# ignaschuemer7/soft-actor-critic

Hardware: NVIDIA B200
Metric: SAC updates/s (higher is better)
Workload: dtype f32

## Files before the change

### soft-actor-critic_b200/csrc/sacx.cu

```cuda
#include "../../include/sacx.h"

#include <cuda_runtime.h>

#include <cmath>
#include <cstdlib>
#include <cstring>
#include <string>
#include <vector>

#include "sacx_engine.cuh"
#include "sacx_per.cuh"

namespace sacx {

thread_local std::string g_err;
int fail(int code, const std::string& msg) {
  g_err = msg;
  return code;
}

constexpr int STAGE_ROWS = 4096;

struct Ring {
  int O, A, n_agents, W;
// ... 435 lines not shown
              if (pass == 1)
                ok = ok && tc_encode(enc, &g.maps.c[j], e->d_tc_scratch + r.part, n_ld, (uint64_t)t.splits * m_pad, n_ld, 32, TC_BM, 0, NA, sstride);
            }
            t.idesc = (1u << 4) | (2u << 7) | (2u << 10) | ((uint32_t)t.a_mn << 15) | ((uint32_t)t.b_mn << 16) |
                      ((uint32_t)(t.n_mma >> 3) << 17) | ((uint32_t)(TC_BM >> 4) << 24);
            t.tile0 = tiles; t.ntiles = t.m_tiles * t.splits;
            tiles += t.ntiles;
          }
          g.p.tiles_per_agent = tiles;
          g.p.total_tiles = tiles * (int)NA;
          g.grid = std::max(1, std::min(g.p.total_tiles, e->n_sms));
        }
        need = std::max(need, so);
      }
    }
    if (!ok) return off("cuTensorMapEncodeTiled rejected an operand layout");
    if (pass == 0) {
      sstride = (uint64_t)((need + 63) / 64 * 64 + 64);
      e->tc_scratch_floats = (size_t)sstride * NA;
      SACX_CUDA(cudaMalloc((void**)&e->d_tc_scratch, e->tc_scratch_floats * sizeof(float)));
      SACX_CUDA(cudaMemset(e->d_tc_scratch, 0, e->tc_scratch_floats * sizeof(float)));
    }
  }
  return SACX_OK;
}

static int engine_setup_rp_tma(Engine* e) {
  if (!e->rp) return SACX_OK;
  RpProgram& P = e->h_prog;
  Plan& plan = e->h_plans[PLAN_RP];
  void* fn = nullptr;
  cudaDriverEntryPointQueryResult qres;
  const bool have = cudaGetDriverEntryPoint("cuTensorMapEncodeTiled", &fn, cudaEnableDefault, &qres) == cudaSuccess && fn;
  std::vector<CUtensorMap> maps(P.n_jobs + 2 * plan.n_ops);
  memset(maps.data(), 0, sizeof(CUtensorMap) * maps.size());
  bool ok = have;
  for (int j = 0; ok && j < P.n_jobs; ++j) {
    const RpJob& jb = P.jobs[j];
    if (!jb.tma) continue;
    cuuint64_t dims[2], strides[1] = {(cuuint64_t)jb.w_ld * 4};
    cuuint32_t box[2], estr[2] = {1, 1};
    box[0] = 32; box[1] = 32;
    if (!jb.bkm) { dims[0] = jb.K; dims[1] = jb.N; }
    else { dims[0] = jb.N; dims[1] = jb.K; }
    ok = ((TcEncodeFn)fn)(&maps[j], CU_TENSOR_MAP_DATA_TYPE_FLOAT32, 2, e->arena + jb.w, dims, strides, box, estr, CU_TENSOR_MAP_INTERLEAVE_NONE,
                          CU_TENSOR_MAP_SWIZZLE_128B, CU_TENSOR_MAP_L2_PROMOTION_L2_128B, CU_TENSOR_MAP_FLOAT_OOB_FILL_NONE) == CUDA_SUCCESS;
  }
  if (!ok) { for (int j = 0; j < P.n_jobs; ++j) P.jobs[j].tma = 0; cudaGetLastError(); }
  const char* dw_env = getenv("SACX_RP_DW_TMA");
  bool ok_dw = have && !(dw_env && atoi(dw_env) == 0);
  for (int k = 0; k < plan.n_ops; ++k) { plan.ops[k].i[2] = 0; plan.ops[k].i[3] = 0; }
  for (int k = 0; ok_dw && k < plan.n_ops; ++k) {
    Op& o = plan.ops[k];
    if (o.type != OP_GEMM || o.epi != EPI_DW || o.a_sm != 1 || o.b_sn != 1 || (o.a & 3) || (o.b & 3) || (o.a_sk & 3) || (o.b_sk & 3)) continue;
    if (o.K > RP_DW_MAXK || o.cfg != 0) continue;
    for (int w = 0; ok_dw && w < 2; ++w) {
      cuuint64_t dims[2] = {(cuuint64_t)(w ? o.N : o.M), (cuuint64_t)o.K}, strides[1] = {(cuuint64_t)(w ? o.b_sk : o.a_sk) * 4};
      cuuint32_t box[2] = {32, (cuuint32_t)RP_DW_CHUNK}, estr[2] = {1, 1};
      ok_dw = ((TcEncodeFn)fn)(&maps[P.n_jobs + 2 * k + w], CU_TENSOR_MAP_DATA_TYPE_FLOAT32, 2, e->arena + (w ? o.b : o.a), dims, strides, box, estr,
                               CU_TENSOR_MAP_INTERLEAVE_NONE, CU_TENSOR_MAP_SWIZZLE_128B, CU_TENSOR_MAP_L2_PROMOTION_L2_128B,
                               CU_TENSOR_MAP_FLOAT_OOB_FILL_NONE) == CUDA_SUCCESS;
    }
    if (ok_dw) { o.i[2] = P.n_jobs + 2 * k + 1; o.i[3] = P.n_jobs + 2 * k + 2; }
  }
  if (!ok_dw) { for (int k = 0; k < plan.n_ops; ++k) { plan.ops[k].i[2] = 0; plan.ops[k].i[3] = 0; } cudaGetLastError(); }
  const char* vec_env = getenv("SACX_RP_DW_VEC");
  if (ok_dw && !(vec_env && atoi(vec_env) == 0)) {
    for (int k = 0; k < plan.n_ops; ++k) {
      Op& o = plan.ops[k];
      o.i[5] = 0;
      if (o.type == OP_GEMM && o.epi == EPI_DW && o.i[3] > 0 && o.M == 1 && o.K <= RP_DWV_MAXK && o.N >= 64 && !(o.flags & DW_ATOMIC) && o.i[0] <= 1) {
        o.i[5] = 1; o.tiles_n = (o.N + RP_DWV_COLS - 1) / RP_DWV_COLS; o.ntiles = o.tiles_n;
      }
    }
    int widest = 0;
    for (int ph = 0; ph < plan.n_phases; ++ph) {
      Phase& p = plan.phases[ph];
      p.ntiles = 0;
      for (int k = p.op0; k < p.op0 + p.nops; ++k) { plan.ops[k].tile0 = p.ntiles; p.ntiles += plan.ops[k].ntiles; }
      widest = std::max(widest, p.ntiles);
    }
    e->rp_grid = std::min(e->n_sms, std::max(e->rp_grid, widest));
  }
  if (e->d_rp_maps) { cudaFree(e->d_rp_maps); e->d_rp_maps = nullptr; }
  bool up = cudaMalloc(&e->d_rp_maps, sizeof(CUtensorMap) * maps.size()) == cudaSuccess;
  up = up && cudaMemcpy(e->d_rp_maps, maps.data(), sizeof(CUtensorMap) * maps.size(), cudaMemcpyHostToDevice) == cudaSuccess;
  if (!up) {
    for (int j = 0; j < P.n_jobs; ++j) P.jobs[j].tma = 0;
    for (int k = 0; k < plan.n_ops; ++k) { plan.ops[k].i[2] = 0; plan.ops[k].i[3] = 0; }
    if (e->d_rp_maps) { cudaFree(e->d_rp_maps); e->d_rp_maps = nullptr; }
    cudaGetLastError();
  }
  SACX_CUDA(cudaMemcpy(e->d_prog, &e->h_prog, sizeof(RpProgram), cudaMemcpyHostToDevice));
  return SACX_OK;
}

// ... 1126 lines not shown
```

### soft-actor-critic_b200/csrc/sacx_engine.cuh

```cuda
#pragma once
#include <cuda_runtime.h>

#include <algorithm>
#include <cstddef>
#include <cstdio>
#include <cstring>
#include <string>
#include <vector>

#include "sacx_kernels.cuh"
#include "sacx_rowpar.cuh"
#include "sacx_tc.cuh"

namespace sacx {

extern thread_local std::string g_err;
int fail(int code, const std::string& msg);
#define SACX_CUDA(call)                                                                        \
  do {                                                                                         \
    cudaError_t e__ = (call);                                                                  \
    if (e__ != cudaSuccess)                                                                    \
      return fail(SACX_ERR_CUDA, std::string(#call) + ": " + cudaGetErrorString(e__));         \
  } while (0)

// ... 749 lines not shown
    if (L - 2 - k >= 0) {
      const int l = L - 1 - k;
      pb.add(gemm_da(n, l, delta[l], ldd(l), delta[l - 1], ldd(l - 1), as.aux(l - 1), as.ld[l - 1]));
    }
    const int lw = L - k;
    if (lw >= 1 && !(skip_head_dw && lw == L))
      pb.add(gemm_dw(n, lw, opt, flags, delta[lw], ldd(lw), as.h[lw - 1], as.ld[lw - 1], is_critic));
    if (k == bwd_stages(n) - 1) pb.add(gemm_dw(n, 0, opt, flags, delta[0], ldd(0), x, ld_x, is_critic));
  }

  bool rowpar_eligible(std::string& why) const {
    const char* env = getenv("SACX_ROWPAR");
    if (env && atoi(env) == 0) { why = "disabled by SACX_ROWPAR=0"; return false; }
    if (cfg.n_agents != 1) { why = "population mode"; return false; }
    if (cfg.dp_world > 1) { why = "data-parallel mode"; return false; }
    { std::string w; if (tc_wanted(w)) { why = "large batch runs the tensor-core path"; return false; } }
    if (cfg.batch_size > 512 && !(env && atoi(env) == 1)) { why = "batch above 512: the tile-parallel kernel is faster"; return false; }
    if (pi.L() < 2 || q1.L() < 2) { why = "fewer than two hidden layers"; return false; }
    if (act_needs_z(pi.act_h) || act_needs_z(q1.act_h)) { why = "hidden activation needs saved pre-activations"; return false; }
    if (cfg.act_dim > RP_MAXA) { why = "action dimension above 8"; return false; }
    if (2 * cfg.obs_dim + cfg.act_dim + 2 > 256) { why = "observation wider than 123"; return false; }
    for (const NetLayout* n : {&pi, &q1})
      for (int l = 1; l <= n->L(); ++l)
        if (n->dims[l] != 64 && n->dims[l] != 128 && n->dims[l] != 256) { why = "hidden width not 64/128/256"; return false; }
    if (2 * (q1.L() + 1) + (pi.L() + 1) + 1 > RP_MAX_DW_OPS) { why = "network too deep"; return false; }
    return true;
  }

  bool build_rowpar(PB& pb) {
    RpProgram& P = h_prog;
    memset(&P, 0, sizeof P);
    const int O = cfg.obs_dim, A = cfg.act_dim, Lq = q1.L(), Lp = pi.L();
    bool overflow = false;
    int wmax = 0;
    auto step = [&](int row_op) {
      if (P.n_steps_a + P.n_steps_c >= RP_MAX_STEPS) { overflow = true; return; }
      RpStep& st = P.steps[P.n_steps_a + P.n_steps_c];
      st.row_op = row_op; st.job0 = P.n_jobs; st.njobs = 0; st.load0 = P.n_loads; st.nloads = 0;
    };
    auto cur = [&]() -> RpStep& { return P.steps[P.n_steps_a + P.n_steps_c]; };
    auto add_job = [&](const RpJob& j) {
      if (P.n_jobs >= RP_MAX_JOBS) { overflow = true; return; }
      const int NS = j.N / RP_CS;
      RpJob jj = j;
      jj.tma = (rp_tma && NS == 32 && (j.w_ld % 4) == 0 && (j.w % 4) == 0 && j.K <= 256) ? 1 : 0;
      jj.map = P.n_jobs;
      P.jobs[P.n_jobs++] = jj; cur().njobs++;
      const int cp_floats = j.bkm ? j.K * NS : NS * (j.Kp + 4);
      const int tma_floats = j.bkm ? j.K * 32 : ((j.K + 31) / 32) * 1024;
      wmax = std::max(wmax, jj.tma ? tma_floats : cp_floats);
    };
    auto add_load = [&](i64 off, int ld, int K, int abuf) {
      if (P.n_loads >= RP_MAX_LOADS) { overflow = true; return; }
      P.loads[P.n_loads++] = RpLoad{off, ld, K, abuf, 0}; cur().nloads++;
    };
    auto fwd = [&](const NetLayout& n, int l, i64 wshift, int a_src, const ActSet& as, int slot) {
      RpJob j; memset(&j, 0, sizeof j);
      j.bkm = 0; j.a_src = a_src; j.K = n.dims[l]; j.Kp = (j.K + 7) & ~7; j.N = n.dims[l + 1]; j.act = n.act_h;
      j.ns_log2 = j.N == 256 ? 5 : (j.N == 128 ? 4 : 3);
      j.w = n.W[l] + wshift; j.w_ld = j.K; j.bias = n.b[l] + wshift; j.out = as.h[l]; j.out_ld = as.ld[l]; j.aux = -1; j.proj_w = -1;
      if (l == n.L() - 1) {
        j.proj_J = n.dims[n.L() + 1]; j.proj_slot = slot; j.proj_w = n.W[n.L()] + wshift; j.proj_sj = n.dims[n.L()]; j.proj_sn = 1;
      }
      return j;
    };
    auto bwd = [&](const NetLayout& n, int l, int a_src, const ActSet& as, const i64* delta, int da_slot) {
      RpJob j; memset(&j, 0, sizeof j);
      j.bkm = 1; j.a_src = a_src; j.K = n.dims[l + 1]; j.Kp = j.K; j.N = n.dims[l]; j.act = n.act_h;
      j.ns_log2 = j.N == 256 ? 5 : (j.N == 128 ? 4 : 3);
      j.w = n.W[l]; j.w_ld = n.dims[l]; j.bias = -1; j.aux = as.h[l - 1]; j.aux_ld = as.ld[l - 1];
      j.out = delta[l - 1]; j.out_ld = rup4(n.dims[l]); j.proj_w = -1;
      if (da_slot >= 0) { j.proj_J = A; j.proj_slot = da_slot; j.proj_w = n.W[0] + O; j.proj_sj = 1; j.proj_sn = n.dims[0]; }
      return j;
    };
    const i64 tsh = T0 - q1.begin;
    step(RPR_GATHER);
    add_job(fwd(pi, 0, 0, RPS_XS2, a_pit, RPP_PI_T));
    add_job(fwd(pi, 0, 0, RPS_XSA, a_pia, RPP_PI_A));
    for (int c = 0; c < 2; ++c) add_job(fwd(c ? q2 : q1, 0, 0, RPS_XSA, a_q[c], RPP_Q1 + c));
    P.n_steps_a++;
    for (int l = 1; l < std::max(Lp, Lq); ++l) {
      step(RPR_NONE);
      if (l < Lp) {
        add_load(a_pit.h[l - 1], a_pit.ld[l - 1], pi.dims[l], 0); add_job(fwd(pi, l, 0, 0, a_pit, RPP_PI_T));
        add_load(a_pia.h[l - 1], a_pia.ld[l - 1], pi.dims[l], 1); add_job(fwd(pi, l, 0, 1, a_pia, RPP_PI_A));
      }
      if (l < Lq)
        for (int c = 0; c < 2; ++c) {
          add_load(a_q[c].h[l - 1], a_q[c].ld[l - 1], q1.dims[l], 2 + c);
          add_job(fwd(c ? q2 : q1, l, 0, 2 + c, a_q[c], RPP_Q1 + c));
        }
      P.n_steps_a++;
    }
    step(RPR_PI_HEADS);
    for (int c = 0; c < 2; ++c) add_job(fwd(c ? q2 : q1, 0, tsh, RPS_XS2, a_qt[c], RPP_QT1 + c));
    P.n_steps_a++;
    for (int l = 1; l < Lq; ++l) {
      step(RPR_NONE);
      for (int c = 0; c < 2; ++c) {
        add_load(a_qt[c].h[l - 1], a_qt[c].ld[l - 1], q1.dims[l], c);
        add_job(fwd(c ? q2 : q1, l, tsh, c, a_qt[c], RPP_QT1 + c));
      }
      P.n_steps_a++;
    }
    step(RPR_TARGET_CRITIC);
    for (int c = 0; c < 2; ++c) {
      add_load(a_q[c].h[Lq - 1], a_q[c].ld[Lq - 1], q1.dims[Lq], 2 + c);
      add_job(bwd(c ? q2 : q1, Lq - 1, 2 + c, a_q[c], d_q[c], -1));
    }
    P.n_steps_a++;
    for (int l = Lq - 2; l >= 1; --l) {
      step(RPR_NONE);
      for (int c = 0; c < 2; ++c) {
        add_load(d_q[c][l], rup4(q1.dims[l + 1]), q1.dims[l + 1], c);
        add_job(bwd(c ? q2 : q1, l, c, a_q[c], d_q[c], -1));
      }
      P.n_steps_a++;
    }
    step(RPR_RELOAD);
    for (int c = 0; c < 2; ++c) add_job(fwd(c ? q2 : q1, 0, 0, RPS_XPI, a_q[c], RPP_Q1 + c));
    P.n_steps_c++;
    for (int l = 1; l < Lq; ++l) {
      step(RPR_NONE);
      for (int c = 0; c < 2; ++c) {
        add_load(a_q[c].h[l - 1], a_q[c].ld[l - 1], q1.dims[l], c);
        add_job(fwd(c ? q2 : q1, l, 0, c, a_q[c], RPP_Q1 + c));
      }
      P.n_steps_c++;
    }
    step(RPR_ACTOR_Q);
    for (int c = 0; c < 2; ++c) {
      add_load(a_q[c].h[Lq - 1], a_q[c].ld[Lq - 1], q1.dims[Lq], 2 + c);
      add_job(bwd(c ? q2 : q1, Lq - 1, 2 + c, a_q[c], d_q[c], Lq - 1 == 1 ? RPP_DA1 + c : -1));
    }
    P.n_steps_c++;
    for (int l = Lq - 2; l >= 1; --l) {
      step(RPR_NONE);
      for (int c = 0; c < 2; ++c) {
        add_load(d_q[c][l], rup4(q1.dims[l + 1]), q1.dims[l + 1], c);
        add_job(bwd(c ? q2 : q1, l, c, a_q[c], d_q[c], l == 1 ? RPP_DA1 + c : -1));
      }
      P.n_steps_c++;
    }
    step(RPR_PI_BWD);
    add_load(a_pia.h[Lp - 1], a_pia.ld[Lp - 1], pi.dims[Lp], 0);
    add_job(bwd(pi, Lp - 1, 0, a_pia, d_p, -1));
    P.n_steps_c++;
    for (int l = Lp - 2; l >= 1; --l) {
      step(RPR_NONE);
      add_load(d_p[l], rup4(pi.dims[l + 1]), pi.dims[l + 1], 1);
      add_job(bwd(pi, l, 1, a_pia, d_p, -1));
      P.n_steps_c++;
    }
    if (overflow) { rp_why = "program tables too small"; return false; }
    P.O = O; P.A = A; P.Hq = q1.dims[Lq]; P.Hpi = pi.dims[Lp]; P.ld_hq = rup4(P.Hq); P.ld_hpi = rup4(P.Hpi);
    P.act_q = q1.act_h; P.act_oq = q1.act_o; P.act_pi = pi.act_h; P.act_opi = pi.act_o;
    P.ab_q[0] = 2; P.ab_q[1] = 3; P.ab_pi = 0;
    P.x_sa = x_sa; P.x_s2 = x_s2; P.x_pi = x_pi; P.b_r = b_r; P.b_d = b_d; P.b_idx = b_idx; P.b_eps1 = b_eps1; P.b_eps2 = b_eps2;
    P.b_lp2 = b_lp2; P.b_lp = b_lp; P.b_y = b_y; P.b_ploss = b_ploss; P.b_tz = b_tz; P.b_se = b_se; P.b_mask = b_mask;
    P.b_headz = b_headz; P.b_dhead = b_dhead;
    for (int c = 0; c < 2; ++c) {
      const NetLayout& n = c ? q2 : q1;
      P.b_tq[c] = b_tq[c]; P.b_q[c] = b_q[c]; P.b_qa[c] = b_qa[c]; P.b_dout[c] = b_dout[c]; P.b_loss[c] = b_loss[c];
      P.q_bL[c] = n.b[Lq]; P.q_WL[c] = n.W[Lq]; P.qt_bL[c] = n.b[Lq] + tsh; P.dq_last[c] = d_q[c][Lq - 1];
    }
    P.pi_bL = pi.b[Lp]; P.pi_WL = pi.W[Lp]; P.dp_last = d_p[Lp - 1];
    int hmax = 0;
    for (int l = 1; l <= Lp; ++l) hmax = std::max(hmax, pi.dims[l]);
    for (int l = 1; l <= Lq; ++l) hmax = std::max(hmax, q1.dims[l]);
    P.lda = hmax + 4; P.abuf_floats = RP_RB * P.lda;
    P.ldx = ((O + A + 7) & ~7) + 4;
    P.gldx = ldx;
    P.wslot_floats = ((wmax + 255) & ~255) + 1024;
    int off = 0;
    P.sm_abuf = off; off += RP_NABUF * P.abuf_floats;
    P.sm_xbuf = off; off += 3 * RP_RB * P.ldx;
    off = (off + 255) & ~255;
    P.sm_wslot = off; off += RP_NWSLOT * P.wslot_floats;
    P.sm_red = off; off += RP_RED;
    P.sm_otile = off; P.sm_pw = off;
    off = std::max(off, WSM_FLOATS + CfgSmall::SMEM_FLOATS);
    off = std::max(off, RP_DW_SMEM);
    P.sm_total = off;
    const int J[RPP_N] = {2 * A, 2 * A, 1, 1, 1, 1, A, A};
    int poff = 0;
    for (int i = 0; i < RPP_N; ++i) { P.part_off[i] = poff; poff += RP_CS * RP_RB * J[i]; }
    P.part_stride = (poff + 31) & ~31;
    const bool keep_large = large;
    large = false;
    const int AD = DW_ADAM;
    pb.phase();
    for (int l = Lq - 1; l >= 1; --l)
      for (int c = 0; c < 2; ++c)
        pb.add(gemm_dw(c ? q2 : q1, l, c ? OPT_Q2 : OPT_Q1, AD | DW_POLYAK, d_q[c][l], rup4(q1.dims[l + 1]), a_q[c].h[l - 1], a_q[c].ld[l - 1], true));
    for (int c = 0; c < 2; ++c) {
      pb.add(gemm_dw(c ? q2 : q1, 0, c ? OPT_Q2 : OPT_Q1, AD | DW_POLYAK, d_q[c][0], rup4(q1.dims[1]), x_sa, ldx, true));
      pb.add(gemm_dw(c ? q2 : q1, Lq, c ? OPT_Q2 : OPT_Q1, AD | DW_POLYAK, b_dout[c], 4, a_q[c].h[Lq - 1], a_q[c].ld[Lq - 1], true));
    }
    pb.phase();
    for (int l = Lp - 1; l >= 1; --l) pb.add(gemm_dw(pi, l, OPT_PI, AD, d_p[l], rup4(pi.dims[l + 1]), a_pia.h[l - 1], a_pia.ld[l - 1], false));
    pb.add(gemm_dw(pi, 0, OPT_PI, AD, d_p[0], rup4(pi.dims[1]), x_pi, ldx, false));
    pb.add(gemm_dw(pi, Lp, OPT_PI, AD, b_dhead, 2 * A, a_pia.h[Lp - 1], a_pia.ld[Lp - 1], false));
    pb.add(op_final(1 | 2 | 4 | 8));
    large = keep_large;
    if (pb.overflow || pb.p.n_ops > RP_MAX_DW_OPS) { rp_why = "too many dW ops"; return false; }
    return true;
  }

  int build_plans() {
    h_plans.assign(N_PLANS, Plan());
    auto put = [&](int id, PB& pb) -> int {
      if (pb.overflow) return fail(SACX_ERR_INVALID, "network too deep for the op table (MAX_OPS/MAX_PHASES)");
// ... 77 lines not shown
```

### soft-actor-critic_b200/csrc/sacx_rowpar.cuh

```cuda
#pragma once
#include "sacx_kernels.cuh"

namespace sacx {

constexpr int RP_CS = 8;
constexpr int RP_RB = 16;
constexpr int RP_HMAX = 256;
constexpr int RP_NABUF = 4;
constexpr int RP_NWSLOT = 3;
constexpr int RP_RED = 2048;
constexpr int RP_MAXA = 8;
constexpr int RP_MAX_GROUPS = 32;
constexpr int RP_MAX_JOBS = 40, RP_MAX_STEPS = 28, RP_MAX_LOADS = 48, RP_MAX_DW_OPS = 16;

enum RpRowOp : int { RPR_NONE = 0, RPR_GATHER, RPR_PI_HEADS, RPR_TARGET_CRITIC, RPR_RELOAD, RPR_ACTOR_Q, RPR_PI_BWD };
enum RpSrc : int { RPS_ABUF0 = 0, RPS_XSA = 4, RPS_XS2 = 5, RPS_XPI = 6 };
enum RpSlot : int { RPP_PI_T = 0, RPP_PI_A, RPP_Q1, RPP_Q2, RPP_QT1, RPP_QT2, RPP_DA1, RPP_DA2, RPP_N };

struct RpJob {
  int bkm;
  int a_src;
  int K, Kp, N;
  int ns_log2;
  int act;
  int w_ld;
  int out_ld, aux_ld;
  int proj_J, proj_slot, proj_sj, proj_sn;
  int tma, map;
  i64 w, bias, out, aux, proj_w;
};
struct RpLoad { i64 off; int ld, K, abuf, pad; };
struct RpStep { int row_op, job0, njobs, load0, nloads, pad0, pad1, pad2; };

struct RpProgram {
  int n_steps_a, n_steps_c, n_jobs, n_loads;
  int n_row_groups, pad_g;
  int sm_abuf, sm_xbuf, ldx, sm_wslot, sm_red, sm_otile, sm_pw, sm_total;
  int lda, abuf_floats, wslot_floats, gldx;
  int O, A, Hq, Hpi, ld_hq, ld_hpi, act_q, act_oq, act_pi, act_opi;
  int ab_q[2], ab_pi, part_stride;
  int part_off[RPP_N];
  i64 x_sa, x_s2, x_pi, b_r, b_d, b_idx, b_eps1, b_eps2, b_lp2, b_lp, b_y, b_tq[2], b_q[2], b_qa[2], b_dout[2],
      b_loss[2], b_ploss, b_tz, b_se, b_mask, b_headz, b_dhead;
  i64 pi_bL, pi_WL, q_bL[2], q_WL[2], qt_bL[2];
  i64 dq_last[2], dp_last;
  RpStep steps[RP_MAX_STEPS];
  RpJob jobs[RP_MAX_JOBS];
  RpLoad loads[RP_MAX_LOADS];
};

struct RpRows {
  float r[RP_RB], d[RP_RB], lp2[RP_RB], lp[RP_RB], coef[2][RP_RB];
  float eps1[RP_RB][RP_MAXA], eps2[RP_RB][RP_MAXA], tz[RP_RB][RP_MAXA], se[RP_RB][RP_MAXA], mk[RP_RB][RP_MAXA];
  float hz[RP_RB][2 * RP_MAXA], dh[RP_RB][2 * RP_MAXA];
};

struct RpTrace { unsigned long long* buf; int n, cap; };

#ifdef SACX_DEBUG_HOOKS
#define RP_TRACE(tag) do { if (c.tr->buf && threadIdx.x == 0 && c.tr->n < c.tr->cap) { \
  c.tr->buf[2 * c.tr->n] = (unsigned long long)(tag); c.tr->buf[2 * c.tr->n + 1] = clock64(); c.tr->n++; } } while (0)
#else
// ... 77 lines not shown
    unsigned old, v;
    asm volatile("atom.add.release.gpu.global.u32 %0, [%1], 1;" : "=r"(old) : "l"(counter) : "memory");
    if (mode & 2) {
      if (old + 1 != epoch) {
        do {
          asm volatile("ld.acquire.gpu.global.u32 %0, [%1];" : "=r"(v) : "l"(counter) : "memory");
        } while ((int)(v - epoch) < 0);
      } else {
        asm volatile("fence.acq_rel.gpu;" ::: "memory");
      }
    } else {
      unsigned* flag = counter + 32;
      if (old + 1 == epoch) {
        asm volatile("st.release.gpu.global.u32 [%0], %1;" ::"l"(flag), "r"(epoch) : "memory");
      } else {
        do {
          asm volatile("ld.acquire.gpu.global.u32 %0, [%1];" : "=r"(v) : "l"(flag) : "memory");
        } while ((int)(v - epoch) < 0);
      }
    }
  }
  __syncthreads();
}

__device__ __forceinline__ void rp_issue_job(const RpJob& jb, float* __restrict__ slot, const RpCtx& c, int slot_idx) {
  const RpProgram& P = *c.P;
  const float* __restrict__ base = c.base;
  const int NS = 1 << jb.ns_log2, n0g = c.rank << jb.ns_log2, tid = threadIdx.x, warp = tid >> 5, lane = tid & 31;
  const float* __restrict__ W = base + jb.w;
  float* eps = slot + P.wslot_floats - 1024;
  float* pws = slot + P.wslot_floats - 512;
  const int J = jb.proj_J, cl = jb.ns_log2 - 2;
  const int B = c.args->hp.B;
  if (jb.tma) {
    if (lane == 0) {
      uint64_t* bar = c.wbar + slot_idx;
      const int slabs = (jb.K + 31) >> 5;
      if (warp < slabs) {
        const char* map = reinterpret_cast<const char*>(c.args->rp_maps) + (size_t)jb.map * 128;
        rp_mbar_expect_tx(bar, 4096u);
        if (!jb.bkm) rp_tma_load(slot + warp * 1024, map, bar, 32 * warp, n0g);
        else rp_tma_load(slot + warp * 1024, map, bar, n0g, 32 * warp);
      } else {
        asm volatile("mbarrier.arrive.shared::cta.b64 _, [%0];" ::"r"((uint32_t)__cvta_generic_to_shared(bar)) : "memory");
      }
    }
    if (!jb.bkm) {
      if (tid < (1 << cl)) cp_async16(eps + (tid << 2), base + jb.bias + n0g + (tid << 2), 16);
    } else if (tid < (RP_RB << cl)) {
      const int m = tid >> cl, cc = (tid & ((1 << cl) - 1)) << 2;
      const bool ok = c.row0 + m < B;
      cp_async16(eps + m * NS + cc, ok ? base + jb.aux + (i64)(c.row0 + m) * jb.aux_ld + n0g + cc : base, ok ? 16 : 0);
    }
  } else if (!jb.bkm) {
    const int ldw = jb.Kp + 4;
    const bool vec = ((jb.K & 3) == 0) && ((jb.w & 3) == 0) && ((jb.w_ld & 3) == 0);
    if (vec) {
      const int cpr = jb.Kp >> 2;
      for (int n = warp; n < NS; n += 8) {
        const float* src = W + (i64)(n0g + n) * jb.w_ld;
        float* dst = slot + n * ldw;
        for (int ch = lane; ch < cpr; ch += 32) {
          const int k = ch << 2;
          if (k < jb.K) cp_async16(dst + k, src + k, 16);
          else *reinterpret_cast<float4*>(dst + k) = make_float4(0.f, 0.f, 0.f, 0.f);
        }
      }
    } else {
      for (int n = warp; n < NS; n += 8)
        for (int k = lane; k < jb.Kp; k += 32)
          slot[n * ldw + k] = (k < jb.K) ? __ldcg(W + (i64)(n0g + n) * jb.w_ld + k) : 0.f;
    }
    if (tid < (1 << cl)) cp_async16(eps + (tid << 2), base + jb.bias + n0g + (tid << 2), 16);
  } else {
    const int sh = 5 - jb.ns_log2;
    const int ch = (tid & ((1 << cl) - 1)) << 2;
    const float* src = W + n0g + ch + (i64)(tid >> cl) * jb.w_ld;
    const i64 sstep = (i64)(256 >> cl) * jb.w_ld;
    for (int k = tid >> cl; k < jb.K; k += 256 >> cl, src += sstep) {
      const int sw = ((k & 3) >> sh) << 3;
      cp_async16(slot + k * NS + (ch ^ sw), src, 16);
    }
    if (tid < (RP_RB << cl)) {
      const int m = tid >> cl, cc = (tid & ((1 << cl) - 1)) << 2;
      const bool ok = c.row0 + m < B;
      cp_async16(eps + m * NS + cc, ok ? base + jb.aux + (i64)(c.row0 + m) * jb.aux_ld + n0g + cc : base, ok ? 16 : 0);
    }
  }
  if (J > 0) {
    if (jb.proj_sn == 1) {
      const int i = tid - 128;
      if (i >= 0 && i < (J << cl)) {
        const int j = i >> cl, cc = (i & ((1 << cl) - 1)) << 2;
        cp_async16(pws + j * NS + cc, base + jb.proj_w + (i64)j * jb.proj_sj + n0g + cc, 16);
      }
    } else {
      for (int i = tid; i < J * NS; i += 256)
        rp_cp_async4(pws + i, base + jb.proj_w + (i64)(i >> jb.ns_log2) * jb.proj_sj + (i64)(n0g + (i & (NS - 1))) * jb.proj_sn);
    }
  }
}

__device__ __forceinline__ void rp_issue_load(const RpLoad& ld, float* __restrict__ abuf, int lda, const float* __restrict__ base, int row0, int B) {
  const int warp = threadIdx.x >> 5, lane = threadIdx.x & 31, cpr = ld.K >> 2;
#pragma unroll
  for (int h = 0; h < 2; ++h) {
// ... 65 lines not shown
        rp_mma3(c0, c1, c2, a, b);
        ++ks;
      }
    }
  }
  for (; ks + 1 < ks1; ks += 2) {
    const float a[4] = {rp_lds(a0p + ao), rp_lds(a1p + ao), rp_lds(a0p + ao + 16u), rp_lds(a1p + ao + 16u)};
    const float b[2] = {rp_lds(bp + bo), rp_lds(bp + bo + b4)};
    const float a2[4] = {rp_lds(a0p + ao + 32u), rp_lds(a1p + ao + 32u), rp_lds(a0p + ao + 48u), rp_lds(a1p + ao + 48u)};
    const float b2[2] = {rp_lds(bp + bo + bstep), rp_lds(bp + bo + bstep + b4)};
    rp_mma3(c0, c1, c2, a, b);
    rp_mma3(d0, d1, d2, a2, b2);
    ao += 64u; bo += 2u * bstep;
  }
  if (ks < ks1) {
    const float a[4] = {rp_lds(a0p + ao), rp_lds(a1p + ao), rp_lds(a0p + ao + 16u), rp_lds(a1p + ao + 16u)};
    const float b[2] = {rp_lds(bp + bo), rp_lds(bp + bo + b4)};
    rp_mma3(c0, c1, c2, a, b);
  }
  const int RS = NS + 8;
  float* r = red + kg * 16 * RS;
  float acc[4];
#pragma unroll
  for (int q = 0; q < 4; ++q) acc[q] = ((c0[q] + d0[q]) + (c1[q] + d1[q])) + (c2[q] + d2[q]);
  *reinterpret_cast<float2*>(r + g * RS + n0 + 2 * t) = make_float2(acc[0], acc[1]);
  *reinterpret_cast<float2*>(r + (g + 8) * RS + n0 + 2 * t) = make_float2(acc[2], acc[3]);
}

__device__ __forceinline__ void rp_job(const RpJob& jb, const RpCtx& c, int wslot_idx) {
  RP_SMEM;
  const RpProgram& P = *c.P;
  const int tid = threadIdx.x, NS = 1 << jb.ns_log2, n0g = c.rank << jb.ns_log2, RS = NS + 8, KG = 64 >> jb.ns_log2;
  const int B = c.args->hp.B;
  const float* As;
  int lda;
  if (jb.a_src < RP_NABUF) { As = smem_raw + P.sm_abuf + jb.a_src * P.abuf_floats; lda = P.lda; }
  else { As = smem_raw + P.sm_xbuf + (jb.a_src - RPS_XSA) * RP_RB * P.ldx; lda = P.ldx; }
  const float* Bs = smem_raw + P.sm_wslot + wslot_idx * P.wslot_floats;
  const float* eps = Bs + P.wslot_floats - 1024;
  const float* pws = Bs + P.wslot_floats - 512;
  float* red = smem_raw + P.sm_red;
  RP_TRACE(4500);
  rp_job_math(jb, rp_saddr(As), lda, rp_saddr(Bs), red);
  RP_TRACE(4600);
  __syncthreads();
  RP_TRACE(4650);
  const int e = tid * 2, m = e >> jb.ns_log2, n = e & (NS - 1);
  if (e < RP_RB * NS) {
    float2 s = make_float2(0.f, 0.f);
    for (int q = 0; q < KG; ++q) {
      const float2 p = *reinterpret_cast<const float2*>(red + (q * 16 + m) * RS + n);
      s.x += p.x; s.y += p.y;
    }
    float2 v;
    if (!jb.bkm) {
      const float2 bb = *reinterpret_cast<const float2*>(eps + n);
      v = make_float2(act_fwd(jb.act, s.x + bb.x), act_fwd(jb.act, s.y + bb.y));
    } else {
      const float2 ax = *reinterpret_cast<const float2*>(eps + m * NS + n);
      v = make_float2(s.x * act_dz(jb.act, ax.x), s.y * act_dz(jb.act, ax.y));
    }
    if (c.row0 + m < B && jb.out >= 0) *reinterpret_cast<float2*>(c.base + jb.out + (i64)(c.row0 + m) * jb.out_ld + n0g + n) = v;
    const int J = jb.proj_J;
    if (J > 0) {
      const int lpr = NS >> 1, r = (tid & 31) & (lpr - 1);
      float* dst = c.part + P.part_off[jb.proj_slot] + (c.rank * RP_RB + m) * J;
      if (J == 1) {
        const float2 w = *reinterpret_cast<const float2*>(pws + n);
        float p1 = fmaf(v.x, w.x, v.y * w.y);
        for (int o = lpr >> 1; o > 0; o >>= 1) p1 += __shfl_xor_sync(0xffffffffu, p1, o);
        if (r == 0) dst[0] = p1;
      } else
      for (int j0 = 0; j0 < J; j0 += 8) {
        float p[8];
#pragma unroll
        for (int jj = 0; jj < 8; ++jj) {
          p[jj] = 0.f;
          if (j0 + jj < J) {
            const float2 w = *reinterpret_cast<const float2*>(pws + (j0 + jj) * NS + n);
            p[jj] = fmaf(v.x, w.x, v.y * w.y);
          }
        }
        for (int o = lpr >> 1; o > 0; o >>= 1) {
#pragma unroll
          for (int jj = 0; jj < 8; ++jj) p[jj] += __shfl_xor_sync(0xffffffffu, p[jj], o);
        }
#pragma unroll
        for (int jj = 0; jj < 8; ++jj)
          if (j0 + jj < J && r == ((j0 + jj) & (lpr - 1))) dst[j0 + jj] = p[jj];
      }
    }
  }
}

struct RpParts { float v[RP_CS]; };
__device__ __forceinline__ void rp_load_parts(const RpCtx& c, int slot, int J, int m, int j, RpParts& o) {
  const float* p = c.part + c.P->part_off[slot] + m * J + j;
#pragma unroll
  for (int r = 0; r < RP_CS; ++r) o.v[r] = __ldcg(p + r * RP_RB * J);
}
__device__ __forceinline__ float rp_add_parts(const RpParts& o) {
  float s = 0.f;
#pragma unroll
  for (int r = 0; r < RP_CS; ++r) s += o.v[r];
  return s;
}
__device__ __forceinline__ float rp_sum8(float v) {
  v += __shfl_xor_sync(0xffffffffu, v, 1);
  v += __shfl_xor_sync(0xffffffffu, v, 2);
  v += __shfl_xor_sync(0xffffffffu, v, 4);
  return v;
}

struct RpLaunch { i64 pushes, upd0, oldest_slot; unsigned long long rng_seed; unsigned rng_agent, pad; };

template <int MAXE>
__device__ __forceinline__ void rp_gather_rows(const RpCtx& c, const i64* __restrict__ slots, const float* __restrict__ ring) {
  RP_SMEM;
  const RunArgs& a = *c.args;
  const RpProgram& P = *c.P;
  RpRows& R = *c.R;
  const int tid = threadIdx.x, O = P.O, A = P.A, ldx = P.ldx;
// ... 776 lines not shown
```

Measured before the change: 9811.

## Pair matching row-parallel forward jobs to share one weight-slot stage

Row-parallel program builder now merges two compatible forward GEMM jobs (policy target/action, q1/q2, target q1/q2) into one paired job. A pair either shares one weight slice or stages both weight slices, plus both biases, into a single slot via TMA or cp.async. The job then runs the math and epilogue twice over separate reduction buffers. This halves the number of job steps and their barriers/weight-slot turnovers per layer, at the cost of larger shared-memory reduction and weight slots, a two-pass program build to size slot capacity, and doubled TMA map tables.

```diff
diff --git a/soft-actor-critic_b200/csrc/sacx.cu b/soft-actor-critic_b200/csrc/sacx.cu
--- a/soft-actor-critic_b200/csrc/sacx.cu
+++ b/soft-actor-critic_b200/csrc/sacx.cu
@@ -491,7 +491,8 @@
   void* fn = nullptr;
   cudaDriverEntryPointQueryResult qres;
   const bool have = cudaGetDriverEntryPoint("cuTensorMapEncodeTiled", &fn, cudaEnableDefault, &qres) == cudaSuccess && fn;
-  std::vector<CUtensorMap> maps(P.n_jobs + 2 * plan.n_ops);
+  const int nj = 2 * P.n_jobs;
+  std::vector<CUtensorMap> maps(nj + 2 * plan.n_ops);
   memset(maps.data(), 0, sizeof(CUtensorMap) * maps.size());
   bool ok = have;
   for (int j = 0; ok && j < P.n_jobs; ++j) {
@@ -502,8 +503,10 @@
     box[0] = 32; box[1] = 32;
     if (!jb.bkm) { dims[0] = jb.K; dims[1] = jb.N; }
     else { dims[0] = jb.N; dims[1] = jb.K; }
-    ok = ((TcEncodeFn)fn)(&maps[j], CU_TENSOR_MAP_DATA_TYPE_FLOAT32, 2, e->arena + jb.w, dims, strides, box, estr, CU_TENSOR_MAP_INTERLEAVE_NONE,
-                          CU_TENSOR_MAP_SWIZZLE_128B, CU_TENSOR_MAP_L2_PROMOTION_L2_128B, CU_TENSOR_MAP_FLOAT_OOB_FILL_NONE) == CUDA_SUCCESS;
+    for (int h = 0; ok && h <= (jb.pair && jb.w2_off > 0 ? 1 : 0); ++h)
+      ok = ((TcEncodeFn)fn)(&maps[h ? jb.map2 : jb.map], CU_TENSOR_MAP_DATA_TYPE_FLOAT32, 2, e->arena + (h ? jb.w2 : jb.w), dims, strides, box, estr,
+                            CU_TENSOR_MAP_INTERLEAVE_NONE, CU_TENSOR_MAP_SWIZZLE_128B, CU_TENSOR_MAP_L2_PROMOTION_L2_128B,
+                            CU_TENSOR_MAP_FLOAT_OOB_FILL_NONE) == CUDA_SUCCESS;
   }
   if (!ok) { for (int j = 0; j < P.n_jobs; ++j) P.jobs[j].tma = 0; cudaGetLastError(); }
   const char* dw_env = getenv("SACX_RP_DW_TMA");
@@ -516,11 +519,11 @@
     for (int w = 0; ok_dw && w < 2; ++w) {
       cuuint64_t dims[2] = {(cuuint64_t)(w ? o.N : o.M), (cuuint64_t)o.K}, strides[1] = {(cuuint64_t)(w ? o.b_sk : o.a_sk) * 4};
       cuuint32_t box[2] = {32, (cuuint32_t)RP_DW_CHUNK}, estr[2] = {1, 1};
-      ok_dw = ((TcEncodeFn)fn)(&maps[P.n_jobs + 2 * k + w], CU_TENSOR_MAP_DATA_TYPE_FLOAT32, 2, e->arena + (w ? o.b : o.a), dims, strides, box, estr,
+      ok_dw = ((TcEncodeFn)fn)(&maps[nj + 2 * k + w], CU_TENSOR_MAP_DATA_TYPE_FLOAT32, 2, e->arena + (w ? o.b : o.a), dims, strides, box, estr,
                                CU_TENSOR_MAP_INTERLEAVE_NONE, CU_TENSOR_MAP_SWIZZLE_128B, CU_TENSOR_MAP_L2_PROMOTION_L2_128B,
                                CU_TENSOR_MAP_FLOAT_OOB_FILL_NONE) == CUDA_SUCCESS;
     }
-    if (ok_dw) { o.i[2] = P.n_jobs + 2 * k + 1; o.i[3] = P.n_jobs + 2 * k + 2; }
+    if (ok_dw) { o.i[2] = nj + 2 * k + 1; o.i[3] = nj + 2 * k + 2; }
   }
   if (!ok_dw) { for (int k = 0; k < plan.n_ops; ++k) { plan.ops[k].i[2] = 0; plan.ops[k].i[3] = 0; } cudaGetLastError(); }
   const char* vec_env = getenv("SACX_RP_DW_VEC");
diff --git a/soft-actor-critic_b200/csrc/sacx_engine.cuh b/soft-actor-critic_b200/csrc/sacx_engine.cuh
--- a/soft-actor-critic_b200/csrc/sacx_engine.cuh
+++ b/soft-actor-critic_b200/csrc/sacx_engine.cuh
@@ -805,23 +805,47 @@
     memset(&P, 0, sizeof P);
     const int O = cfg.obs_dim, A = cfg.act_dim, Lq = q1.L(), Lp = pi.L();
     bool overflow = false;
-    int wmax = 0;
+    int wmax = 0, red = 0, wcap = 0;
     auto step = [&](int row_op) {
       if (P.n_steps_a + P.n_steps_c >= RP_MAX_STEPS) { overflow = true; return; }
       RpStep& st = P.steps[P.n_steps_a + P.n_steps_c];
       st.row_op = row_op; st.job0 = P.n_jobs; st.njobs = 0; st.load0 = P.n_loads; st.nloads = 0;
     };
     auto cur = [&]() -> RpStep& { return P.steps[P.n_steps_a + P.n_steps_c]; };
+    auto tma_ok = [&](const RpJob& j, i64 w) { return rp_tma && j.N / RP_CS == 32 && (j.w_ld % 4) == 0 && (w % 4) == 0 && j.K <= 256; };
+    auto slice_floats = [&](const RpJob& j, bool tma) {
+      const int NS = j.N / RP_CS;
+      if (tma) return j.bkm ? j.K * 32 : ((j.K + 31) / 32) * 1024;
+      return j.bkm ? j.K * NS : NS * (j.Kp + 4);
+    };
+    auto pair_w2_off = [&](const RpJob& j, bool tma) {
+      if (!tma) return (slice_floats(j, false) + 3) & ~3;
+      return (std::max(slice_floats(j, true), slice_floats(j, false)) + 255) & ~255;
+    };
     auto add_job = [&](const RpJob& j) {
       if (P.n_jobs >= RP_MAX_JOBS) { overflow = true; return; }
       const int NS = j.N / RP_CS;
       RpJob jj = j;
-      jj.tma = (rp_tma && NS == 32 && (j.w_ld % 4) == 0 && (j.w % 4) == 0 && j.K <= 256) ? 1 : 0;
-      jj.map = P.n_jobs;
+      const bool sep = j.pair && j.w2 != j.w;
+      jj.tma = (tma_ok(j, j.w) && (!sep || tma_ok(j, j.w2))) ? 1 : 0;
+      jj.map = 2 * P.n_jobs; jj.map2 = 2 * P.n_jobs + 1;
+      jj.w2_off = sep ? pair_w2_off(j, jj.tma) : 0;
       P.jobs[P.n_jobs++] = jj; cur().njobs++;
-      const int cp_floats = j.bkm ? j.K * NS : NS * (j.Kp + 4);
-      const int tma_floats = j.bkm ? j.K * 32 : ((j.K + 31) / 32) * 1024;
-      wmax = std::max(wmax, jj.tma ? tma_floats : cp_floats);
+      wmax = std::max(wmax, jj.w2_off + (sep ? jj.w2_off : slice_floats(j, jj.tma)));
+      red = std::max(red, (1 + j.pair) * (64 / NS) * RP_RB * (NS + 8));
+    };
+    auto add_pair = [&](const RpJob& a, const RpJob& b) {
+      const bool shared = a.w == b.w && a.bias == b.bias && a.proj_w == b.proj_w;
+      bool ok = wcap > 0 && !a.bkm && !b.bkm && a.K == b.K && a.N == b.N && a.act == b.act && a.w_ld == b.w_ld &&
+                a.out_ld == b.out_ld && a.proj_J == b.proj_J && (shared || a.proj_J == 0);
+      if (ok && !shared) {
+        const bool tma = tma_ok(a, a.w) && tma_ok(a, b.w);
+        ok = 2 * pair_w2_off(a, tma) <= wcap && (!tma || 2 * ((a.K + 31) / 32) <= 8);
+      }
+      if (!ok) { add_job(a); add_job(b); return; }
+      RpJob j = a;
+      j.pair = 1; j.a_src2 = b.a_src; j.out2 = b.out; j.proj_slot2 = b.proj_slot; j.w2 = b.w; j.bias2 = b.bias;
+      add_job(j);
     };
     auto add_load = [&](i64 off, int ld, int K, int abuf) {
       if (P.n_loads >= RP_MAX_LOADS) { overflow = true; return; }
@@ -847,84 +871,86 @@
       return j;
     };
     const i64 tsh = T0 - q1.begin;
-    step(RPR_GATHER);
-    add_job(fwd(pi, 0, 0, RPS_XS2, a_pit, RPP_PI_T));
-    add_job(fwd(pi, 0, 0, RPS_XSA, a_pia, RPP_PI_A));
-    for (int c = 0; c < 2; ++c) add_job(fwd(c ? q2 : q1, 0, 0, RPS_XSA, a_q[c], RPP_Q1 + c));
-    P.n_steps_a++;
-    for (int l = 1; l < std::max(Lp, Lq); ++l) {
-      step(RPR_NONE);
-      if (l < Lp) {
-        add_load(a_pit.h[l - 1], a_pit.ld[l - 1], pi.dims[l], 0); add_job(fwd(pi, l, 0, 0, a_pit, RPP_PI_T));
-        add_load(a_pia.h[l - 1], a_pia.ld[l - 1], pi.dims[l], 1); add_job(fwd(pi, l, 0, 1, a_pia, RPP_PI_A));
-      }
-      if (l < Lq)
+    auto emit = [&]() {
+      step(RPR_GATHER);
+      add_pair(fwd(pi, 0, 0, RPS_XS2, a_pit, RPP_PI_T), fwd(pi, 0, 0, RPS_XSA, a_pia, RPP_PI_A));
+      add_pair(fwd(q1, 0, 0, RPS_XSA, a_q[0], RPP_Q1), fwd(q2, 0, 0, RPS_XSA, a_q[1], RPP_Q2));
+      P.n_steps_a++;
+      for (int l = 1; l < std::max(Lp, Lq); ++l) {
+        step(RPR_NONE);
+        if (l < Lp) {
+          add_load(a_pit.h[l - 1], a_pit.ld[l - 1], pi.dims[l], 0);
+          add_load(a_pia.h[l - 1], a_pia.ld[l - 1], pi.dims[l], 1);
+          add_pair(fwd(pi, l, 0, 0, a_pit, RPP_PI_T), fwd(pi, l, 0, 1, a_pia, RPP_PI_A));
+        }
+        if (l < Lq) {
+          for (int c = 0; c < 2; ++c) add_load(a_q[c].h[l - 1], a_q[c].ld[l - 1], q1.dims[l], 2 + c);
+          add_pair(fwd(q1, l, 0, 2, a_q[0], RPP_Q1), fwd(q2, l, 0, 3, a_q[1], RPP_Q2));
+        }
+        P.n_steps_a++;
+      }
+      step(RPR_PI_HEADS);
+      add_pair(fwd(q1, 0, tsh, RPS_XS2, a_qt[0], RPP_QT1), fwd(q2, 0, tsh, RPS_XS2, a_qt[1], RPP_QT2));
+      P.n_steps_a++;
+      for (int l = 1; l < Lq; ++l) {
+        step(RPR_NONE);
+        for (int c = 0; c < 2; ++c) add_load(a_qt[c].h[l - 1], a_qt[c].ld[l - 1], q1.dims[l], c);
+        add_pair(fwd(q1, l, tsh, 0, a_qt[0], RPP_QT1), fwd(q2, l, tsh, 1, a_qt[1], RPP_QT2));
+        P.n_steps_a++;
+      }
+      step(RPR_TARGET_CRITIC);
+      for (int c = 0; c < 2; ++c) {
+        add_load(a_q[c].h[Lq - 1], a_q[c].ld[Lq - 1], q1.dims[Lq], 2 + c);
+        add_job(bwd(c ? q2 : q1, Lq - 1, 2 + c, a_q[c], d_q[c], -1));
+      }
+      P.n_steps_a++;
+      for (int l = Lq - 2; l >= 1; --l) {
+        step(RPR_NONE);
         for (int c = 0; c < 2; ++c) {
-          add_load(a_q[c].h[l - 1], a_q[c].ld[l - 1], q1.dims[l], 2 + c);
-          add_job(fwd(c ? q2 : q1, l, 0, 2 + c, a_q[c], RPP_Q1 + c));
+          add_load(d_q[c][l], rup4(q1.dims[l + 1]), q1.dims[l + 1], c);
+          add_job(bwd(c ? q2 : q1, l, c, a_q[c], d_q[c], -1));
         }
-      P.n_steps_a++;
-    }
-    step(RPR_PI_HEADS);
-    for (int c = 0; c < 2; ++c) add_job(fwd(c ? q2 : q1, 0, tsh, RPS_XS2, a_qt[c], RPP_QT1 + c));
-    P.n_steps_a++;
-    for (int l = 1; l < Lq; ++l) {
-      step(RPR_NONE);
+        P.n_steps_a++;
+      }
+      step(RPR_RELOAD);
+      add_pair(fwd(q1, 0, 0, RPS_XPI, a_q[0], RPP_Q1), fwd(q2, 0, 0, RPS_XPI, a_q[1], RPP_Q2));
+      P.n_steps_c++;
+      for (int l = 1; l < Lq; ++l) {
+        step(RPR_NONE);
+        for (int c = 0; c < 2; ++c) add_load(a_q[c].h[l - 1], a_q[c].ld[l - 1], q1.dims[l], c);
+        add_pair(fwd(q1, l, 0, 0, a_q[0], RPP_Q1), fwd(q2, l, 0, 1, a_q[1], RPP_Q2));
+        P.n_steps_c++;
+      }
+      step(RPR_ACTOR_Q);
       for (int c = 0; c < 2; ++c) {
-        add_load(a_qt[c].h[l - 1], a_qt[c].ld[l - 1], q1.dims[l], c);
-        add_job(fwd(c ? q2 : q1, l, tsh, c, a_qt[c], RPP_QT1 + c));
-      }
-      P.n_steps_a++;
-    }
-    step(RPR_TARGET_CRITIC);
-    for (int c = 0; c < 2; ++c) {
-      add_load(a_q[c].h[Lq - 1], a_q[c].ld[Lq - 1], q1.dims[Lq], 2 + c);
-      add_job(bwd(c ? q2 : q1, Lq - 1, 2 + c, a_q[c], d_q[c], -1));
-    }
-    P.n_steps_a++;
-    for (int l = Lq - 2; l >= 1; --l) {
-      step(RPR_NONE);
-      for (int c = 0; c < 2; ++c) {
-        add_load(d_q[c][l], rup4(q1.dims[l + 1]), q1.dims[l + 1], c);
-        add_job(bwd(c ? q2 : q1, l, c, a_q[c], d_q[c], -1));
-      }
-      P.n_steps_a++;
-    }
-    step(RPR_RELOAD);
-    for (int c = 0; c < 2; ++c) add_job(fwd(c ? q2 : q1, 0, 0, RPS_XPI, a_q[c], RPP_Q1 + c));
-    P.n_steps_c++;
-    for (int l = 1; l < Lq; ++l) {
-      step(RPR_NONE);
-      for (int c = 0; c < 2; ++c) {
-        add_load(a_q[c].h[l - 1], a_q[c].ld[l - 1], q1.dims[l], c);
-        add_job(fwd(c ? q2 : q1, l, 0, c, a_q[c], RPP_Q1 + c));
+        add_load(a_q[c].h[Lq - 1], a_q[c].ld[Lq - 1], q1.dims[Lq], 2 + c);
+        add_job(bwd(c ? q2 : q1, Lq - 1, 2 + c, a_q[c], d_q[c], Lq - 1 == 1 ? RPP_DA1 + c : -1));
       }
       P.n_steps_c++;
-    }
-    step(RPR_ACTOR_Q);
-    for (int c = 0; c < 2; ++c) {
-      add_load(a_q[c].h[Lq - 1], a_q[c].ld[Lq - 1], q1.dims[Lq], 2 + c);
-      add_job(bwd(c ? q2 : q1, Lq - 1, 2 + c, a_q[c], d_q[c], Lq - 1 == 1 ? RPP_DA1 + c : -1));
-    }
-    P.n_steps_c++;
-    for (int l = Lq - 2; l >= 1; --l) {
-      step(RPR_NONE);
-      for (int c = 0; c < 2; ++c) {
-        add_load(d_q[c][l], rup4(q1.dims[l + 1]), q1.dims[l + 1], c);
-        add_job(bwd(c ? q2 : q1, l, c, a_q[c], d_q[c], l == 1 ? RPP_DA1 + c : -1));
-      }
+      for (int l = Lq - 2; l >= 1; --l) {
+        step(RPR_NONE);
+        for (int c = 0; c < 2; ++c) {
+          add_load(d_q[c][l], rup4(q1.dims[l + 1]), q1.dims[l + 1], c);
+          add_job(bwd(c ? q2 : q1, l, c, a_q[c], d_q[c], l == 1 ? RPP_DA1 + c : -1));
+        }
+        P.n_steps_c++;
+      }
+      step(RPR_PI_BWD);
+      add_load(a_pia.h[Lp - 1], a_pia.ld[Lp - 1], pi.dims[Lp], 0);
+      add_job(bwd(pi, Lp - 1, 0, a_pia, d_p, -1));
       P.n_steps_c++;
-    }
-    step(RPR_PI_BWD);
-    add_load(a_pia.h[Lp - 1], a_pia.ld[Lp - 1], pi.dims[Lp], 0);
-    add_job(bwd(pi, Lp - 1, 0, a_pia, d_p, -1));
-    P.n_steps_c++;
-    for (int l = Lp - 2; l >= 1; --l) {
-      step(RPR_NONE);
-      add_load(d_p[l], rup4(pi.dims[l + 1]), pi.dims[l + 1], 1);
-      add_job(bwd(pi, l, 1, a_pia, d_p, -1));
-      P.n_steps_c++;
-    }
+      for (int l = Lp - 2; l >= 1; --l) {
+        step(RPR_NONE);
+        add_load(d_p[l], rup4(pi.dims[l + 1]), pi.dims[l + 1], 1);
+        add_job(bwd(pi, l, 1, a_pia, d_p, -1));
+        P.n_steps_c++;
+      }
+    };
+    emit();
+    wcap = wmax;
+    P.n_steps_a = P.n_steps_c = P.n_jobs = P.n_loads = 0;
+    wmax = red = 0; overflow = false;
+    emit();
     if (overflow) { rp_why = "program tables too small"; return false; }
     P.O = O; P.A = A; P.Hq = q1.dims[Lq]; P.Hpi = pi.dims[Lp]; P.ld_hq = rup4(P.Hq); P.ld_hpi = rup4(P.Hpi);
     P.act_q = q1.act_h; P.act_oq = q1.act_o; P.act_pi = pi.act_h; P.act_opi = pi.act_o;
@@ -950,7 +976,7 @@
     P.sm_xbuf = off; off += 3 * RP_RB * P.ldx;
     off = (off + 255) & ~255;
     P.sm_wslot = off; off += RP_NWSLOT * P.wslot_floats;
-    P.sm_red = off; off += RP_RED;
+    P.sm_red = off; off += red;
     P.sm_otile = off; P.sm_pw = off;
     off = std::max(off, WSM_FLOATS + CfgSmall::SMEM_FLOATS);
     off = std::max(off, RP_DW_SMEM);
diff --git a/soft-actor-critic_b200/csrc/sacx_rowpar.cuh b/soft-actor-critic_b200/csrc/sacx_rowpar.cuh
--- a/soft-actor-critic_b200/csrc/sacx_rowpar.cuh
+++ b/soft-actor-critic_b200/csrc/sacx_rowpar.cuh
@@ -8,7 +8,6 @@
 constexpr int RP_HMAX = 256;
 constexpr int RP_NABUF = 4;
 constexpr int RP_NWSLOT = 3;
-constexpr int RP_RED = 2048;
 constexpr int RP_MAXA = 8;
 constexpr int RP_MAX_GROUPS = 32;
 constexpr int RP_MAX_JOBS = 40, RP_MAX_STEPS = 28, RP_MAX_LOADS = 48, RP_MAX_DW_OPS = 16;
@@ -28,6 +27,8 @@
   int proj_J, proj_slot, proj_sj, proj_sn;
   int tma, map;
   i64 w, bias, out, aux, proj_w;
+  int pair, a_src2, proj_slot2, map2, w2_off, pad_p;
+  i64 w2, bias2, out2;
 };
 struct RpLoad { i64 off; int ld, K, abuf, pad; };
 struct RpStep { int row_op, job0, njobs, load0, nloads, pad0, pad1, pad2; };
@@ -171,21 +172,26 @@
   float* pws = slot + P.wslot_floats - 512;
   const int J = jb.proj_J, cl = jb.ns_log2 - 2;
   const int B = c.args->hp.B;
+  const bool sep = jb.pair && jb.w2_off > 0;
   if (jb.tma) {
     if (lane == 0) {
       uint64_t* bar = c.wbar + slot_idx;
       const int slabs = (jb.K + 31) >> 5;
-      if (warp < slabs) {
-        const char* map = reinterpret_cast<const char*>(c.args->rp_maps) + (size_t)jb.map * 128;
+      if (warp < (sep ? 2 * slabs : slabs)) {
+        const bool h = warp >= slabs;
+        const int wt = h ? warp - slabs : warp;
+        const char* map = reinterpret_cast<const char*>(c.args->rp_maps) + (size_t)(h ? jb.map2 : jb.map) * 128;
+        float* dst = slot + (h ? jb.w2_off : 0) + wt * 1024;
         rp_mbar_expect_tx(bar, 4096u);
-        if (!jb.bkm) rp_tma_load(slot + warp * 1024, map, bar, 32 * warp, n0g);
-        else rp_tma_load(slot + warp * 1024, map, bar, n0g, 32 * warp);
+        if (!jb.bkm) rp_tma_load(dst, map, bar, 32 * wt, n0g);
+        else rp_tma_load(dst, map, bar, n0g, 32 * wt);
       } else {
         asm volatile("mbarrier.arrive.shared::cta.b64 _, [%0];" ::"r"((uint32_t)__cvta_generic_to_shared(bar)) : "memory");
       }
     }
     if (!jb.bkm) {
       if (tid < (1 << cl)) cp_async16(eps + (tid << 2), base + jb.bias + n0g + (tid << 2), 16);
+      else if (sep && tid >= 32 && tid < 32 + (1 << cl)) cp_async16(eps + 32 + ((tid - 32) << 2), base + jb.bias2 + n0g + ((tid - 32) << 2), 16);
     } else if (tid < (RP_RB << cl)) {
       const int m = tid >> cl, cc = (tid & ((1 << cl) - 1)) << 2;
       const bool ok = c.row0 + m < B;
@@ -193,24 +199,30 @@
     }
   } else if (!jb.bkm) {
     const int ldw = jb.Kp + 4;
-    const bool vec = ((jb.K & 3) == 0) && ((jb.w & 3) == 0) && ((jb.w_ld & 3) == 0);
-    if (vec) {
-      const int cpr = jb.Kp >> 2;
-      for (int n = warp; n < NS; n += 8) {
-        const float* src = W + (i64)(n0g + n) * jb.w_ld;
-        float* dst = slot + n * ldw;
-        for (int ch = lane; ch < cpr; ch += 32) {
-          const int k = ch << 2;
-          if (k < jb.K) cp_async16(dst + k, src + k, 16);
-          else *reinterpret_cast<float4*>(dst + k) = make_float4(0.f, 0.f, 0.f, 0.f);
+    for (int h = 0; h <= (int)sep; ++h) {
+      const i64 wo = h ? jb.w2 : jb.w;
+      const float* __restrict__ Wh = base + wo;
+      float* sl = slot + (h ? jb.w2_off : 0);
+      const bool vec = ((jb.K & 3) == 0) && ((wo & 3) == 0) && ((jb.w_ld & 3) == 0);
+      if (vec) {
+        const int cpr = jb.Kp >> 2;
+        for (int n = warp; n < NS; n += 8) {
+          const float* src = Wh + (i64)(n0g + n) * jb.w_ld;
+          float* dst = sl + n * ldw;
+          for (int ch = lane; ch < cpr; ch += 32) {
+            const int k = ch << 2;
+            if (k < jb.K) cp_async16(dst + k, src + k, 16);
+            else *reinterpret_cast<float4*>(dst + k) = make_float4(0.f, 0.f, 0.f, 0.f);
+          }
         }
-      }
-    } else {
-      for (int n = warp; n < NS; n += 8)
-        for (int k = lane; k < jb.Kp; k += 32)
-          slot[n * ldw + k] = (k < jb.K) ? __ldcg(W + (i64)(n0g + n) * jb.w_ld + k) : 0.f;
+      } else {
+        for (int n = warp; n < NS; n += 8)
+          for (int k = lane; k < jb.Kp; k += 32)
+            sl[n * ldw + k] = (k < jb.K) ? __ldcg(Wh + (i64)(n0g + n) * jb.w_ld + k) : 0.f;
+      }
     }
     if (tid < (1 << cl)) cp_async16(eps + (tid << 2), base + jb.bias + n0g + (tid << 2), 16);
+    else if (sep && tid >= 32 && tid < 32 + (1 << cl)) cp_async16(eps + 32 + ((tid - 32) << 2), base + jb.bias2 + n0g + ((tid - 32) << 2), 16);
   } else {
     const int sh = 5 - jb.ns_log2;
     const int ch = (tid & ((1 << cl) - 1)) << 2;
@@ -342,62 +354,72 @@
   const RpProgram& P = *c.P;
   const int tid = threadIdx.x, NS = 1 << jb.ns_log2, n0g = c.rank << jb.ns_log2, RS = NS + 8, KG = 64 >> jb.ns_log2;
   const int B = c.args->hp.B;
-  const float* As;
-  int lda;
-  if (jb.a_src < RP_NABUF) { As = smem_raw + P.sm_abuf + jb.a_src * P.abuf_floats; lda = P.lda; }
-  else { As = smem_raw + P.sm_xbuf + (jb.a_src - RPS_XSA) * RP_RB * P.ldx; lda = P.ldx; }
   const float* Bs = smem_raw + P.sm_wslot + wslot_idx * P.wslot_floats;
   const float* eps = Bs + P.wslot_floats - 1024;
   const float* pws = Bs + P.wslot_floats - 512;
   float* red = smem_raw + P.sm_red;
+  const int red_half = KG * 16 * RS;
   RP_TRACE(4500);
-  rp_job_math(jb, rp_saddr(As), lda, rp_saddr(Bs), red);
+#pragma unroll 1
+  for (int h = 0; h <= jb.pair; ++h) {
+    const int src = h ? jb.a_src2 : jb.a_src;
+    const float* As;
+    int lda;
+    if (src < RP_NABUF) { As = smem_raw + P.sm_abuf + src * P.abuf_floats; lda = P.lda; }
+    else { As = smem_raw + P.sm_xbuf + (src - RPS_XSA) * RP_RB * P.ldx; lda = P.ldx; }
+    rp_job_math(jb, rp_saddr(As), lda, rp_saddr(Bs + (h ? jb.w2_off : 0)), red + h * red_half);
+  }
   RP_TRACE(4600);
   __syncthreads();
   RP_TRACE(4650);
   const int e = tid * 2, m = e >> jb.ns_log2, n = e & (NS - 1);
   if (e < RP_RB * NS) {
-    float2 s = make_float2(0.f, 0.f);
-    for (int q = 0; q < KG; ++q) {
-      const float2 p = *reinterpret_cast<const float2*>(red + (q * 16 + m) * RS + n);
-      s.x += p.x; s.y += p.y;
-    }
-    float2 v;
-    if (!jb.bkm) {
-      const float2 bb = *reinterpret_cast<const float2*>(eps + n);
-      v = make_float2(act_fwd(jb.act, s.x + bb.x), act_fwd(jb.act, s.y + bb.y));
-    } else {
-      const float2 ax = *reinterpret_cast<const float2*>(eps + m * NS + n);
-      v = make_float2(s.x * act_dz(jb.act, ax.x), s.y * act_dz(jb.act, ax.y));
-    }
-    if (c.row0 + m < B && jb.out >= 0) *reinterpret_cast<float2*>(c.base + jb.out + (i64)(c.row0 + m) * jb.out_ld + n0g + n) = v;
-    const int J = jb.proj_J;
-    if (J > 0) {
-      const int lpr = NS >> 1, r = (tid & 31) & (lpr - 1);
-      float* dst = c.part + P.part_off[jb.proj_slot] + (c.rank * RP_RB + m) * J;
-      if (J == 1) {
-        const float2 w = *reinterpret_cast<const float2*>(pws + n);
-        float p1 = fmaf(v.x, w.x, v.y * w.y);
-        for (int o = lpr >> 1; o > 0; o >>= 1) p1 += __shfl_xor_sync(0xffffffffu, p1, o);
-        if (r == 0) dst[0] = p1;
-      } else
-      for (int j0 = 0; j0 < J; j0 += 8) {
-        float p[8];
-#pragma unroll
-        for (int jj = 0; jj < 8; ++jj) {
-          p[jj] = 0.f;
-          if (j0 + jj < J) {
-            const float2 w = *reinterpret_cast<const float2*>(pws + (j0 + jj) * NS + n);
-            p[jj] = fmaf(v.x, w.x, v.y * w.y);
+#pragma unroll 1
+    for (int h = 0; h <= jb.pair; ++h) {
+      const float* rh = red + h * red_half;
+      float2 s = make_float2(0.f, 0.f);
+      for (int q = 0; q < KG; ++q) {
+        const float2 p = *reinterpret_cast<const float2*>(rh + (q * 16 + m) * RS + n);
+        s.x += p.x; s.y += p.y;
+      }
+      float2 v;
+      if (!jb.bkm) {
+        const float2 bb = *reinterpret_cast<const float2*>(eps + (h && jb.w2_off ? 32 : 0) + n);
+        v = make_float2(act_fwd(jb.act, s.x + bb.x), act_fwd(jb.act, s.y + bb.y));
+      } else {
+        const float2 ax = *reinterpret_cast<const float2*>(eps + m * NS + n);
+        v = make_float2(s.x * act_dz(jb.act, ax.x), s.y * act_dz(jb.act, ax.y));
+      }
+      const i64 out = h ? jb.out2 : jb.out;
+      if (c.row0 + m < B && out >= 0) *reinterpret_cast<float2*>(c.base + out + (i64)(c.row0 + m) * jb.out_ld + n0g + n) = v;
+      const int J = jb.proj_J;
+      if (J > 0) {
+        const int lpr = NS >> 1, r = (tid & 31) & (lpr - 1);
+        float* dst = c.part + P.part_off[h ? jb.proj_slot2 : jb.proj_slot] + (c.rank * RP_RB + m) * J;
+        if (J == 1) {
+          const float2 w = *reinterpret_cast<const float2*>(pws + n);
+          float p1 = fmaf(v.x, w.x, v.y * w.y);
+          for (int o = lpr >> 1; o > 0; o >>= 1) p1 += __shfl_xor_sync(0xffffffffu, p1, o);
+          if (r == 0) dst[0] = p1;
+        } else
+        for (int j0 = 0; j0 < J; j0 += 8) {
+          float p[8];
+#pragma unroll
+          for (int jj = 0; jj < 8; ++jj) {
+            p[jj] = 0.f;
+            if (j0 + jj < J) {
+              const float2 w = *reinterpret_cast<const float2*>(pws + (j0 + jj) * NS + n);
+              p[jj] = fmaf(v.x, w.x, v.y * w.y);
+            }
           }
+          for (int o = lpr >> 1; o > 0; o >>= 1) {
+#pragma unroll
+            for (int jj = 0; jj < 8; ++jj) p[jj] += __shfl_xor_sync(0xffffffffu, p[jj], o);
+          }
+#pragma unroll
+          for (int jj = 0; jj < 8; ++jj)
+            if (j0 + jj < J && r == ((j0 + jj) & (lpr - 1))) dst[j0 + jj] = p[jj];
         }
-        for (int o = lpr >> 1; o > 0; o >>= 1) {
-#pragma unroll
-          for (int jj = 0; jj < 8; ++jj) p[jj] += __shfl_xor_sync(0xffffffffu, p[jj], o);
-        }
-#pragma unroll
-        for (int jj = 0; jj < 8; ++jj)
-          if (j0 + jj < J && r == ((j0 + jj) & (lpr - 1))) dst[j0 + jj] = p[jj];
       }
     }
   }
```

Measured after the change: 10200 (median of 6 runs). 4.0% higher.
